# mushroomfire/mdapy

Hardware: AMD Instinct MI355X
Metric: atoms/sec for neighbor+CNA on 10M-atom FCC Cu; 1/2/4/8-GPU scaling (higher is better)
Workload: dtype f64 (CNA pair tests: f32 filter + f64 finish, labels exact); 1 GPU; FCC Cu a=3.615, 136^3 cells per GPU (10061824 atoms/GPU, 10061824 total), build_neighbor(rc=0.854a=3.08721, max_neigh=16) + fixed-cutoff CNA as one C-ABI call (mdh_build_neighbor_fcna: lists and labels), positions resident in HBM; atoms_per_gpu=10061824, max_neigh=16, parallelism=single, world_size_checked=1, launched_by=single process

## Files before the change

include/mdapy_amd.h:

```cpp
#ifndef MDAPY_AMD_H
#define MDAPY_AMD_H

#include <stdint.h>

#ifdef __cplusplus
extern "C" {
#endif

#define MDH_HOST 0
#define MDH_DEVICE 1

#define MDH_OK 0
#define MDH_ERR_BOX (-1)
#define MDH_ERR_HIP (-2)
#define MDH_ERR_ARG (-3)
#define MDH_ERR_NOMEM (-4)

const char *mdh_last_error(void);
int mdh_version(void);
int mdh_device_count(void);
int mdh_set_device(int device);
int mdh_warm(void);
int mdh_min_max_i32(const int *v, int64_t n, int *min_max2, int space, void *stream);
int mdh_dense_codes_i32(const int *v, int64_t n, int low, int span, int *codes, int64_t *counts_span, int space, void *stream);
int mdh_release_workspace(void);
int64_t mdh_workspace_bytes(void);
int mdh_prof_enable(int on);
int mdh_prof_reset(void);
int mdh_prof_report(char *buf, int buflen);
int mdh_debug_set_neighbor_variant(int variant);
int mdh_debug_set_indirect(int on);
int mdh_debug_set_slot_grid(int on);
int mdh_debug_slot_grid_counters(int64_t *out4);
int mdh_debug_slot_grid_rule(int ordered, int keyed, int windowed, int row_width, int64_t ncell, int64_t N, int seen, int big, int listed);
int mdh_debug_grid_plan(const int64_t *in24, const double *in6, int *out15);
int mdh_debug_neighbor_plan(int *plan8);
int mdh_debug_lane_plan(const int64_t *in_i, const double *in_d, const int *stats, double *out);
int mdh_debug_run_offset_table(int txy, int tz, unsigned *out3);
int mdh_debug_set_fcna_variant(int variant);
int mdh_debug_track_counters(int on);
int mdh_debug_counters(int64_t *out4);
int mdh_debug_set_rdf_variant(int variant);
int mdh_debug_set_knn_variant(int variant);
int mdh_debug_set_sq_variant(int variant);
int mdh_debug_set_entropy_variant(int variant);
int mdh_debug_set_ptm_order_cap(int cap);
int mdh_debug_image_thresholds(double L, double *out4);

int mdh_parse_table(const char *text, int64_t nbytes, int text_space, int64_t nrows, int ncol, const int *kinds,
                    void *const *columns, int64_t *redo, int64_t redo_cap, int64_t *status4, int space, void *stream);
int mdh_debug_text_pow5(int q, uint64_t *out2);
int mdh_debug_parse_double(const char *s, int64_t len, double *out);
int mdh_scan_sections(const char *text, int64_t nbytes, int text_space, const char *const *words, int nwords, int64_t *first_offset,
// ... 313 lines not shown
```

mdapy_amd/_lib.py:

```python
from __future__ import annotations

import ctypes as C
import os

import numpy as np

_HERE = os.path.dirname(os.path.abspath(__file__))
LIB_PATH = os.path.join(_HERE, "csrc", "libmdapy_amd.so")

HOST, DEVICE = 0, 1
ERR_BOX, ERR_HIP, ERR_ARG, ERR_NOMEM = -1, -2, -3, -4

_lib = None

i64, dbl, cint, vp = C.c_int64, C.c_double, C.c_int, C.c_void_p
ALLOC_ROWS = C.CFUNCTYPE(C.c_int, C.c_void_p, C.c_int64, C.c_int64, C.POINTER(C.POINTER(C.c_int)), C.POINTER(C.POINTER(C.c_double)))

_SIGNATURES = {
    "mdh_last_error": [],
    "mdh_version": [],
    "mdh_device_count": [],
    "mdh_set_device": [cint],
    "mdh_warm": [],
    "mdh_min_max_i32": [vp, i64, vp, cint, vp],
    "mdh_dense_codes_i32": [vp, i64, cint, cint, vp, vp, cint, vp],
    "mdh_release_workspace": [],
    "mdh_workspace_bytes": [],
    "mdh_prof_enable": [cint],
    "mdh_prof_reset": [],
    "mdh_prof_report": [vp, cint],
    "mdh_debug_set_neighbor_variant": [cint],
    "mdh_debug_set_indirect": [cint],
    "mdh_debug_set_slot_grid": [cint],
    "mdh_debug_slot_grid_counters": [vp],
    "mdh_debug_slot_grid_rule": [cint, cint, cint, cint, i64, i64, cint, cint, cint],
    "mdh_debug_grid_plan": [vp, vp, vp],
    "mdh_debug_neighbor_plan": [vp],
    "mdh_debug_lane_plan": [vp, vp, vp, vp],
    "mdh_debug_run_offset_table": [cint, cint, vp],
    "mdh_debug_set_fcna_variant": [cint],
    "mdh_debug_track_counters": [cint],
    "mdh_debug_counters": [vp],
    "mdh_debug_set_rdf_variant": [cint],
    "mdh_debug_set_knn_variant": [cint],
    "mdh_debug_set_sq_variant": [cint],
    "mdh_debug_set_entropy_variant": [cint],
    "mdh_debug_set_ptm_order_cap": [cint],
    "mdh_debug_image_thresholds": [dbl, vp],
    "mdh_parse_table": [vp, i64, cint, i64, cint, vp, vp, vp, i64, vp, cint, vp],
    "mdh_debug_text_pow5": [cint, vp],
    "mdh_debug_parse_double": [C.c_char_p, i64, vp],
    "mdh_scan_sections": [vp, i64, cint, vp, cint, vp, vp, vp],
    "mdh_debug_scan_sections": [vp, i64, vp, cint, vp, vp],
    "mdh_format_table": [i64, cint, vp, vp, vp, vp, vp, vp, i64, vp, vp, cint, vp],
# ... 192 lines not shown
```

mdapy_amd/csrc/neighbor_lane.hip:

```cpp
#include "common.hpp"
#include "grid.hpp"
#include "cna_core.hpp"
#include <algorithm>
#include <cassert>
#include <cmath>
#include <type_traits>
#include <cstdio>
#include <cstdlib>
#include <cstring>

namespace mdh {
namespace lane {

static constexpr int NEUTRAL = img::CELL_NEUTRAL;
static constexpr int NEUTRAL3 = img::NEUTRAL;

struct FastDiv {
    unsigned mul, sh1, sh2, d;
    __device__ __forceinline__ unsigned div(unsigned n) const
    {
        const unsigned t = __umulhi(mul, n);
        return (t + ((n - t) >> sh1)) >> sh2;
    }
};
// ... 28 lines not shown
}
static Shape make_shape(int txy, int tz, int nt1, int nt2)
{
    assert(txy >= 1 && tz >= 1 && (txy + 2) * (txy + 2) * (tz + 2) <= RUN_TABLE_HALO);
    assert(2 * run_offset(txy, tz, 8) <= RUN_TABLE_SPAN);
    Shape s{txy, tz, make_fastdiv((unsigned)nt2), make_fastdiv((unsigned)nt1), (65536u + (unsigned)tz + 1u) / ((unsigned)tz + 2u),
            (65536u + (unsigned)txy + 1u) / ((unsigned)txy + 2u), 0u, 0u, 0u};
    run_offset_table(txy, tz, &s.ro_lo, &s.ro_hi, &s.ro_bias);
    return s;
}
typedef __attribute__((address_space(3))) unsigned char lds_byte;
typedef int Int4 __attribute__((ext_vector_type(4)));

static thread_local int g_last_plan[8];
static thread_local int g_last_listed = -1;
#ifdef MDH_STAMPS
__device__ unsigned long long g_stamps[65536 * 8];
#define STAMP(k) do { if (tid == 0 && !parent && tile.id < 65536) g_stamps[tile.id * 8 + (k)] = __builtin_amdgcn_s_memtime(); } while (0)
#else
#define STAMP(k) do {} while (0)
#endif

__device__ __forceinline__ void lds_barrier()
{
    asm volatile("s_waitcnt lgkmcnt(0)\n\ts_barrier" ::: "memory");
}

__device__ __forceinline__ int excl_scan_block(int v, int *scratch, int *total)
{
    const int lane = threadIdx.x & 63, w = threadIdx.x >> 6;
// ... 93 lines not shown
                 "s_waitcnt lgkmcnt(2)\n\t" MDH_CAND2("v100", "v101", "v102", "v104", "v105", "v106")
                 "ds_read_b128 v[100:103], %[a] offset:128\n\t"
                 "ds_read_b128 v[104:107], %[a] offset:144\n\t"
                 "s_waitcnt lgkmcnt(2)\n\t" MDH_CAND2("v108", "v109", "v110", "v112", "v113", "v114")
                 "ds_read_b128 v[108:111], %[a] offset:160\n\t"
                 "ds_read_b128 v[112:115], %[a] offset:176\n\t"
                 "s_waitcnt lgkmcnt(2)\n\t" MDH_CAND2("v100", "v101", "v102", "v104", "v105", "v106")
                 "s_waitcnt lgkmcnt(0)\n\t" MDH_CAND2("v108", "v109", "v110", "v112", "v113", "v114")
                 : [m] "=&v"(m), [w] "+v"(w)
                 : [a] "v"(a), [sx] "v"(sx), [sy] "v"(sy), [sz] "v"(sz), [negc] "v"(negc)
                 : "memory", "v100", "v101", "v102", "v103", "v104", "v105", "v106", "v107", "v108", "v109", "v110", "v111", "v112", "v113",
                   "v114", "v115", "v116", "v117", "v118", "v119", "v120", "v121");
    mask = m;
}
#undef MDH_CAND2
__device__ __forceinline__ int run_slots(int len)
{
    return (len + 3) & ~3;
}

__device__ __forceinline__ bool sqrt_fast_ok(double x)
{
    return x >= 0x1p-767 && x < 0x1p+1000;
}
__device__ __forceinline__ bool sqrt_fast_ok4(const double (&x)[4])
{
    const unsigned h0 = (unsigned)__double2hiint(x[0]), h1 = (unsigned)__double2hiint(x[1]), h2 = (unsigned)__double2hiint(x[2]),
                   h3 = (unsigned)__double2hiint(x[3]);
    const unsigned lo = min(min(min(h0, h1), h2), h3), hi = max(max(max(h0, h1), h2), h3);
    return lo >= (256u << 20) && hi < (2023u << 20);
// ... 3 lines not shown
    const double y = __builtin_amdgcn_rsq(x);
    double g = x * y;
    double h = y * 0.5;
    const double r = __builtin_fma(-h, g, 0.5);
    g = __builtin_fma(g, r, g);
    h = __builtin_fma(h, r, h);
    const double d0 = __builtin_fma(-g, g, x);
    g = __builtin_fma(d0, h, g);
    const double d1 = __builtin_fma(-g, g, x);
    return __builtin_fma(d1, h, g);
}

template <bool SELF, bool TRI>
__device__ __forceinline__ unsigned scan_run_f64(const double2 *__restrict__ lxy, const double *__restrict__ lz,
                                                 const unsigned short *__restrict__ lsh, const DBox &b, double rcsq, int k0, int len,
                                                 int li, double xi, double yi, double zi)
{
    unsigned m = 0;
    const int S = run_slots(len);
    for (int j = 0; j < S; ++j) {
        const int k = k0 + j;
        bool h = false;
        if (j < len) {
            const double2 cj = lxy[k];
            const double d2 = exact_d2<TRI ? 2 : 1>(b, cj.x, cj.y, lz[k], xi, yi, zi, TRI ? 0 : lsh[k]);
            h = (d2 <= rcsq) && (!SELF || k != li);
        }
        m = m + m + (h ? 1u : 0u);
    }
    return m;
}

template <int NN, class Index>
__device__ __forceinline__ int lane_fcna_f32(Index index_of, const float4 *__restrict__ f4, float negc, float W)
{
    float ux[NN], uy[NN], uz[NN];
#pragma unroll
    for (int a = 0; a < NN; ++a) {
        const float4 c = f4[index_of(a)];
        ux[a] = c.x; uy[a] = c.y; uz[a] = c.z;
// ... 65 lines not shown
__device__ __forceinline__ CellGrid::Packed load_record(const CellGrid::Packed *__restrict__ pk, const IndirectSrc &src, int q, int coded)
{
    if (!IND)
        return pk[q];
    return load_atom(src, src.order[q], coded);
}

template <bool COUNT, bool TRI, bool LOOP, bool FCNA, bool TK8, bool IND = false, bool SLOT = false>
__global__ __launch_bounds__(NW * 64, (TK8 && (!FCNA || !LOOP)) ? 16 / NW : 1) void k_neighbor_lane(
    const CellGrid::Packed *__restrict__ pk, const int *__restrict__ cell_start, DBox b,
    Grid g, double rc, float negc, float W, int *__restrict__ verlet, double *__restrict__ dist, int *__restrict__ nn,
    int M, int write_pads, int cap, int *__restrict__ flags, unsigned char *__restrict__ tile_flag, int nt0,
    int nt1, int nt2, Shape ts, const int *__restrict__ tile_list, const int *__restrict__ n_live, int list_mode,
    int *__restrict__ max_count, int *__restrict__ flagged, const int *__restrict__ parent, int parent_nt2, int nsub,
    int flag_slot, int *__restrict__ pattern, int *__restrict__ cna_todo, int jt0, int rw, int tile_base, int *__restrict__ listed_sink,
    int cen_lo, int cen_hi, IndirectSrc isrc, int slot_hi)
{
    const int TXY = ts.txy, TZ = ts.tz;
    const int coded = IND ? flags[4] : 0;
    const int HXY = TXY + 2, HZ = TZ + 2, NH = HXY * HXY * HZ;

    extern __shared__ __attribute__((aligned(16))) unsigned char smem[];
    const int tid = threadIdx.x, lane = tid & 63;
    typedef typename std::conditional<TK8, unsigned char, unsigned short>::type Ticket;
    constexpr int JB = TK8 ? 5 : 8;
    float4 *f4 = reinterpret_cast<float4 *>(smem);
    double2 *lxy = reinterpret_cast<double2 *>(f4 + cap);
    double *lz = reinterpret_cast<double *>(lxy + cap);
    unsigned *cen = reinterpret_cast<unsigned *>(lz + cap);
    unsigned short *lsh = reinterpret_cast<unsigned short *>(cen + CEN_CAP);
    Ticket *tk = reinterpret_cast<Ticket *>(lsh + cap + (cap & 1));
    const unsigned f4_lds = (unsigned)(unsigned long)(lds_byte *)smem;
    const int TKS = ticket_row(M, false);
    const int wstride = max(rw * TKS, 256 / (int)sizeof(Ticket));
    auto hc = [&](int t) -> unsigned & { return reinterpret_cast<unsigned *>(tk + (size_t)(t >> 6) * wstride)[t & 63]; };
    __shared__ unsigned hr[NW * 64 + 2];
    __shared__ int scan_tmp[NW];
    __shared__ int s_flag[4];

    const double rcsq = rc * rc, pad = rc + 1.0;
    const double cw = rc;
    int vmax = 0;

    const int nlive = parent ? min(*n_live, nt0 * nt1 * parent_nt2) * nsub : ((list_mode && tile_list) ? *n_live : nt0 * nt1 * nt2);
    const int per = (nlive + 7) / 8;
// ... 85 lines not shown
    };
    for (int jt = jt0 + (int)(blockIdx.x >> 3); jt < per; jt += (int)(gridDim.x >> 3)) {
        const int slot = (int)(blockIdx.x & 7) * per + jt;
        if (slot >= nlive)
            break;
        const Tile tile = tile_of(slot);
        STAMP(0);
        Halo cur = halo_of(tile);
#ifdef MDH_STAMPS
        asm volatile("" : "+v"(cur.src), "+v"(cur.cnt));
        STAMP(1);
#endif
        double pa[4], pb[4], pc[4];
        int pd[4], pm[4];
        request(cur, pa, pb, pc, pd, pm);
        if (flags[0] != 0)
            return;
        const int tile_id = tile.id, T0 = tile.T0, T1 = tile.T1, T2 = tile.T2;
        const int cnt = cur.cnt, src = cur.src, img = cur.img, hz = cur.hz;
        const bool edge = cur.edge, centre_cell = cur.centre;
        if (tid == 0) { s_flag[0] = 0; s_flag[1] = 0; s_flag[2] = 0; s_flag[3] = 0; }
        hc(tid) = (unsigned)cnt;

        int total2;
        const int off2 = excl_scan_block(cnt | (centre_cell ? cnt << 16 : 0), scan_tmp, &total2);
        const int total = total2 & 0xffff, ncentres = total2 >> 16;
        const int off0 = off2 & 0xffff, coff = off2 >> 16;
        bool ok = !(total > cap || ncentres > CEN_CAP);
        const bool no_centres = ncentres == 0;
        if (no_centres) ok = false;
        if (SLOT && (img & 64)) s_flag[2] = 1;
        STAMP(2);
        if (ok && tid < NH && hz >= 1 && hz <= HZ - 2) {
            const unsigned k0 = (unsigned)off0 - hc(tid - 1), len = hc(tid - 1) + (unsigned)cnt + hc(tid + 1);
            hr[tid] = k0 | (len << 16);
            if (len > (TK8 ? 32u : 96u)) s_flag[2] = 1;
            if (TK8 && len > 12u) s_flag[3] = 1;
        }
        if (ok && cnt > 0) {
            double X0, Y0, Z0, XS, YS, ZS;
            const bool plain = !TRI && tile.interior;
            const int code0 = plain ? NEUTRAL3 : combine_codes(img, img::ATOM_NEUTRAL);
            if (TRI) {
                const double f0 = (double)(T0 - 1) * (cw / b.thick[0]) + (double)img::axis(code0, 0);
                const double f1 = (double)(T1 - 1) * (cw / b.thick[1]) + (double)img::axis(code0, 1);
                const double f2 = (double)(T2 - 1) * (cw / b.thick[2]) + (double)img::axis(code0, 2);
                XS = b.o[0] + f0 * b.h[0] + f1 * b.h[3] + f2 * b.h[6];
                YS = b.o[1] + f0 * b.h[1] + f1 * b.h[4] + f2 * b.h[7];
                ZS = b.o[2] + f0 * b.h[2] + f1 * b.h[5] + f2 * b.h[8];
                X0 = XS; Y0 = YS; Z0 = ZS;
            } else {
                X0 = b.o[0] + (double)(T0 - 1) * cw; Y0 = b.o[1] + (double)(T1 - 1) * cw; Z0 = b.o[2] + (double)(T2 - 1) * cw;
                if (plain) {
                    XS = X0; YS = Y0; ZS = Z0;
                } else {
                    XS = X0 + b.h[0] * (double)img::axis(code0, 0); YS = Y0 + b.h[4] * (double)img::axis(code0, 1);
                    ZS = Z0 + b.h[8] * (double)img::axis(code0, 2);
                }
            }
            const float flo = (float)(-1.5 * cw);
            const float fhx = (float)(((double)HXY + 1.5) * cw), fhz = (float)(((double)HZ + 1.5) * cw);
            bool general = code0 != NEUTRAL3, far = false;
            auto stage4 = [&](int k, const double (&a)[4], const double (&bb)[4], const double (&c)[4], const int (&d)[4], const int (&m)[4]) {
#pragma unroll
                for (int v = 0; v < 4; ++v) {
                    if (k + v < cnt) {
                        int code = code0;
                        float ux, uy, uz;
                        if (TRI) {
// ... 8 lines not shown
                                far = far || !(s0 >= -1.5 && s0 <= (double)HXY + 1.5 && s1 >= -1.5 && s1 <= (double)HXY + 1.5 && s2 >= -1.5 && s2 <= (double)HZ + 1.5);
                            }
                        } else {
                            ux = (float)(a[v] - XS); uy = (float)(bb[v] - YS); uz = (float)(c[v] - ZS);
                        }
                        if (!TRI && m[v] != img::ATOM_NEUTRAL) {
                            code = combine_codes(img, m[v]);
                            ux = (float)((a[v] - b.h[0] * (double)img::axis(code, 0)) - X0);
                            uy = (float)((bb[v] - b.h[4] * (double)img::axis(code, 1)) - Y0);
                            uz = (float)((c[v] - b.h[8] * (double)img::axis(code, 2)) - Z0);
                            general = true;
                        }
                        if (!TRI && edge)
                            far = far || !(ux >= flo && ux <= fhx && uy >= flo && uy <= fhx && uz >= flo && uz <= fhz);
                        const int p = off0 + k + v;
                        f4[p] = make_float4(ux, uy, uz, __int_as_float(d[v]));
                        lxy[p] = make_double2(a[v], bb[v]);
                        lz[p] = c[v];
                        lsh[p] = (unsigned short)code;
                        if (centre_cell) cen[coff + k + v] = (unsigned)p | ((unsigned)tid << 11);
                    }
                }
            };
            if (TK8) {
                for (int k = 0; k < cnt; k += 4) {
                    double a[4], bb[4], c[4];
                    int d[4], m[4];
#pragma unroll
                    for (int v = 0; v < 4; ++v) {
                        if (k == 0) { a[v] = pa[v]; bb[v] = pb[v]; c[v] = pc[v]; d[v] = pd[v]; m[v] = pm[v]; }
                        else {
                            const int kv = min(k + v, cnt - 1);
                            const int q = src + kv + (SLOT && kv >= 4 ? slot_hi : 0);
                            const CellGrid::Packed r = load_record<IND>(pk, isrc, q, coded);
// ... 23 lines not shown
                }
            }
            if (general) s_flag[0] = 1;
            if (far) s_flag[1] = 1;
        }
        __syncthreads();
        STAMP(3);
        if (ok && (s_flag[1] | s_flag[2]))
            ok = false;
        if (!ok && !no_centres && tid == 0) {
            if (tile_flag) tile_flag[tile_id] = 1;
            flagged[atomicAdd(&flags[flag_slot], 1)] = tile_id;
        }
        const bool general_tile = s_flag[0] != 0;
        const bool short_runs = TK8 && s_flag[3] == 0;
        const int wv = tid >> 6;
        Ticket *tkw = tk + (size_t)wv * wstride;
        const int A2 = HXY * HZ;
        auto run_cell = [&](int cbv, int r) {
            const int r3 = (r * 11) >> 5;
            return cbv + __mul24(r3, A2 - 3 * HZ) + __mul24(r, HZ) - (A2 + HZ);
        };
        constexpr unsigned R8 = TRI ? 8u : RUN8_SEL;
        auto run_at = [&](int cbv, unsigned cbk, unsigned sel) {
            return TRI ? run_cell(cbv, (int)sel) : (int)(cbk + __builtin_amdgcn_perm(ts.ro_hi, ts.ro_lo, sel));
        };
        for (int cbase = (int)((unsigned)(wv - jt) & (unsigned)(NW - 1)) * rw; ok && cbase < ncentres; cbase += NW * rw) {
            const int q = cbase + lane;
            const bool mine = lane < rw && q < ncentres;
            int kept = 0, kept8 = 0, cb = 0, id = 0;
            double xi = 0, yi = 0, zi = 0;
            Ticket *my = tkw + (size_t)lane * TKS;
            if (mine) {
                const unsigned cv = cen[q];
                const int li = (int)(cv & 2047u);
                cb = (int)(cv >> 11);
                const float4 s = f4[li];
                constexpr bool WIDE = !TK8;
                unsigned hv[9], mk[9], mk2[WIDE ? 9 : 1], mk3[WIDE ? 9 : 1];
#pragma unroll
                for (int r = 0; r < 9; ++r)
                    hv[r] = hr[cb + ((r / 3 - 1) * HXY + (r % 3 - 1)) * HZ];
                unsigned w = 0x7f7fffffu;
                if (TK8 && short_runs) {
#pragma unroll
                    for (int r = 0; r < 9; ++r) {
                        const int len = (int)(hv[r] >> 16);
                        scan_run12_asm(f4_lds + ((hv[r] & 0xffffu) << 4), s.x, s.y, s.z, negc, mk[r], w);
                        mk[r] = keep_top(mk[r] << 20, len);
                    }
                } else {
#pragma unroll
                    for (int r = 0; r < 9; ++r) {
                        const int len = (int)(hv[r] >> 16), la = WIDE ? min(len, 32) : len;
                        scan_run_asm(f4_lds + ((hv[r] & 0xffffu) << 4), la, s.x, s.y, s.z, negc, mk[r], w);
                        if (TK8)
                            mk[r] = and_not(mk[r] << ((32 - run_slots(la)) & 31), 0x7fffffffu >> ((la - 1) & 31));
                        else mk[r] &= ~0u << (run_slots(la) - la);
                        if (WIDE) {
                            const int lb = min(len - la, 32), lc = len - la - lb;
                            mk2[r] = 0;
                            mk3[r] = 0;
                            if (__builtin_amdgcn_ballot_w64(lb > 0)) {
                                scan_run_asm(f4_lds + (((hv[r] & 0xffffu) + 32u) << 4), lb, s.x, s.y, s.z, negc, mk2[r], w);
                                mk2[r] &= lb > 0 ? ~0u << (run_slots(lb) - lb) : 0u;
                                if (__builtin_amdgcn_ballot_w64(lc > 0)) {
                                    scan_run_asm(f4_lds + (((hv[r] & 0xffffu) + 64u) << 4), lc, s.x, s.y, s.z, negc, mk3[r], w);
                                    mk3[r] &= lc > 0 ? ~0u << (run_slots(lc) - lc) : 0u;
                                }
                            }
// ... 9 lines not shown
                }
                STAMP(4);
                {
                    const double2 ci = lxy[li];
                    xi = ci.x; yi = ci.y; zi = lz[li];
                    if (b.anypbc) {
                        if (TRI || general_tile) {
                            wrap<TRI>(b, xi, yi, zi);
                        } else {
                            if (b.pbc[0]) xi = b.o[0] + (xi - b.o[0]);
                            if (b.pbc[1]) yi = b.o[1] + (yi - b.o[1]);
                            if (b.pbc[2]) zi = b.o[2] + (zi - b.o[2]);
                        }
                    }
                }
                if (__builtin_expect(w <= __float_as_uint(W), 0)) {
#pragma unroll
                    for (int r = 0; r < 9; ++r) {
                        const int k0 = (int)(hv[r] & 0xffffu), len = (int)(hv[r] >> 16), la = WIDE ? min(len, 32) : len;
                        if (r == 4) mk[r] = scan_run_f64<true, TRI>(lxy, lz, lsh, b, rcsq, k0, la, li, xi, yi, zi);
                        else mk[r] = scan_run_f64<false, TRI>(lxy, lz, lsh, b, rcsq, k0, la, li, xi, yi, zi);
                        if (TK8) mk[r] <<= (32 - run_slots(la)) & 31;
                        if (WIDE) {
                            const int lb = min(len - la, 32), lc = len - la - lb;
                            if (r == 4) mk2[r] = scan_run_f64<true, TRI>(lxy, lz, lsh, b, rcsq, k0 + 32, lb, li, xi, yi, zi);
                            else mk2[r] = scan_run_f64<false, TRI>(lxy, lz, lsh, b, rcsq, k0 + 32, lb, li, xi, yi, zi);
                            if (r == 4) mk3[r] = scan_run_f64<true, TRI>(lxy, lz, lsh, b, rcsq, k0 + 64, lc, li, xi, yi, zi);
                            else mk3[r] = scan_run_f64<false, TRI>(lxy, lz, lsh, b, rcsq, k0 + 64, lc, li, xi, yi, zi);
                        }
                    }
                }
                int hits = 0;
#pragma unroll
                for (int r = 0; r < 9; ++r) hits += __builtin_popcount(mk[r]) + (WIDE ? __builtin_popcount(mk2[r]) + __builtin_popcount(mk3[r]) : 0);
                id = __float_as_int(s.w);
                nn[id] = hits;
                if (COUNT) {
                    vmax = max(vmax, hits);
                } else {
                    int sl = 0;
                    auto step = [&](unsigned &m, int jb) {
                        int z;
                        asm("v_ffbh_u32 %0, %1" : "=v"(z) : "v"(m));
                        const int none = z >> 31;
                        const unsigned slot = min((unsigned)(sl | none), (unsigned)M);
                        my[slot] = (Ticket)(jb + z);
                        sl += none + 1;
                        m &= ~(0x80000000u >> (z & 31));
                    };
#pragma unroll
// ... 65 lines not shown
                        for (int u = 0; u < 4; ++u) {
                            const int sx = g0 + u;
                            h[u] = sx < kept;
                            const unsigned t = (tw[sx >> 2] >> (8 * (sx & 3))) & 255u;
                            unsigned r = (sx >= kept - kept8) ? R8 : t >> 5;
                            r = h[u] ? r : 4u;
                            k[u] = (int)(hr[run_at(cb, cbk, r)] & 0xffffu) + (h[u] ? (int)(t & 31u) : 0);
                        }
                        double2 cj[4];
                        double zj[4], d2[4];
                        int nid[4], sh[4];
#pragma unroll
                        for (int u = 0; u < 4; ++u) {
                            cj[u] = lxy[k[u]];
                            zj[u] = lz[k[u]];
                            nid[u] = __float_as_int(f4[k[u]].w);
                            sh[u] = (!TRI && general_tile) ? (int)lsh[k[u]] : 0;
                        }
#pragma unroll
                        for (int u = 0; u < 4; ++u) {
                            if (TRI) d2[u] = exact_d2<2>(b, cj[u].x, cj[u].y, zj[u], xi, yi, zi, 0);
                            else if (general_tile) d2[u] = exact_d2<1>(b, cj[u].x, cj[u].y, zj[u], xi, yi, zi, sh[u]);
                            else d2[u] = exact_d2<0>(b, cj[u].x, cj[u].y, zj[u], xi, yi, zi, 0);
                            d2[u] = h[u] ? d2[u] : 1.0;
                        }
                        const bool slow = !sqrt_fast_ok4(d2);
                        double rr[4];
                        if (__builtin_expect(__builtin_amdgcn_ballot_w64(slow) == 0, 1)) {
#pragma unroll
                            for (int u = 0; u < 4; ++u) rr[u] = sqrt_fast(d2[u]);
                        } else {
// ... 299 lines not shown
    int *flagged2 = sc.alloc_n<int>((size_t)ntiles * (size_t)ll.nsub);
    if (sc.failed())
        return sc.error();
    hipStream_t st = sc.stream();
    if (ll.tiles == LaneLaunch::LIST) {
        hipLaunchKernelGGL(k_tile_live, dim3(grid_for(ntiles, 256)), dim3(256), 0, st, cg.cell_start, cg.g, nt[0], nt[1], nt[2], ts, live, cg.slot_cap);
        MDH_TRY(exclusive_scan_u32(sc, live, slot, ntiles));
        hipLaunchKernelGGL(k_tile_compact, dim3(grid_for(ntiles, 256)), dim3(256), 0, st, live, slot, (int)ntiles, tile_list);
    } else {
        tile_list = nullptr;
    }
    const dim3 grid(ll.grid);
    const size_t lds = (size_t)plan.lds_bytes;
    const int Mi = (int)M, wp = fill_pads ? (rows.ids_only ? 3 : 1) : 0;
    const float negc = -plan.mid;
    const dim3 grid2(SLICE_GRID);
    const Shape ts2 = make_shape(ts.txy, 1, nt[1], ll.nt2b);
    const bool indirect = !cg.pk;
    const lane::IndirectSrc isrc{cg.ix, cg.iy, cg.iz, cg.imv, cg.order};
    const int slot_hi = cg.slot_cap ? (int)(cg.slot_hi - 4) : 0;
#define MDH_LANE_PASS_I(COUNT, TRI, LOOP, FCNA, TK8, IND, SLOT, GRID, JT0, ...)                                                                 \
    do {                                                                                                                                  \
        if (lds > 60 * 1024)                             \
            (void)hipFuncSetAttribute(reinterpret_cast<const void *>(&k_neighbor_lane<COUNT, TRI, LOOP, FCNA, TK8, IND, SLOT>), hipFuncAttributeMaxDynamicSharedMemorySize, (int)lds); \
        hipLaunchKernelGGL((k_neighbor_lane<COUNT, TRI, LOOP, FCNA, TK8, IND, SLOT>), GRID, dim3(NW * 64), lds, st, cg.pk, cg.cell_start, b, \
                           cg.g, rc, negc, plan.T, verlet, dist, nn, Mi, wp, plan.cap, cg.flags, nullptr, __VA_ARGS__, pattern, tf.cna_todo, JT0, plan.rw, ll.tile_base, gs.listed_sink, \
                           ll.cen_lo, ll.cen_hi, isrc, slot_hi); \
    } while (0)
#define MDH_LANE_PASS(COUNT, TRI, LOOP, FCNA, TK8, GRID, JT0, ...)                                                                        \
    do {                                                                                                                                  \
        if (indirect && cg.slot_cap) MDH_LANE_PASS_I(COUNT, TRI, LOOP, FCNA, TK8, true, true, GRID, JT0, __VA_ARGS__);                    \
        else if (indirect) MDH_LANE_PASS_I(COUNT, TRI, LOOP, FCNA, TK8, true, false, GRID, JT0, __VA_ARGS__);                             \
        else MDH_LANE_PASS_I(COUNT, TRI, LOOP, FCNA, TK8, false, false, GRID, JT0, __VA_ARGS__);                                          \
    } while (0)
#define MDH_LANE_LAUNCH(COUNT, TRI, FCNA, TK8)                                                                                            \
    do {                                                                                                                                  \
        if (ll.tiles == LaneLaunch::LIST) {                                                                                               \
            MDH_LANE_PASS(COUNT, TRI, false, FCNA, TK8, grid, 0, nt[0], nt[1], nt[2], ts, tile_list, slot + ntiles, 1, max_count, flagged, nullptr, 0, 1, 2); \
            if (ll.standby)                                                                                                               \
                MDH_LANE_PASS(COUNT, TRI, true, FCNA, TK8, dim3(STANDBY_GRID), ll.per, nt[0], nt[1], nt[2], ts, tile_list, slot + ntiles, 1, max_count, flagged, nullptr, 0, 1, 2); \
        } else {                                                                                                                          \
            MDH_LANE_PASS(COUNT, TRI, false, FCNA, TK8, grid, 0, ll.nt0_run, nt[1], nt[2], ts, nullptr, slot + ntiles, 0, max_count, flagged, nullptr, 0, 1, 2); \
// ... 65 lines not shown
                             (double)p.occupied, (double)p.reason, (double)p.lds_bytes, (double)p.pop, (double)p.over96, (double)p.runs};
    std::copy(lane, lane + 15, out);
    std::copy(hook, hook + 8, out + 15);
    if (p.txy) {
        const LaneLaunch ll = plan_lane_launch(p, in.nc, (int)in_i[13], (int)in_i[14], (int)in_i[15], (int)in_i[16], gs.last_listed);
        const double launch[16] = {(double)ll.nt[0], (double)ll.nt[1], (double)ll.nt[2], (double)ll.ntiles, (double)ll.tiles, (double)ll.tile_base, (double)ll.nt0_run,
                                   (double)ll.per, (double)ll.grid, (double)ll.standby, (double)ll.slice_pass, (double)ll.nsub, (double)ll.nt2b, (double)ll.list_cap,
                                   (double)ll.mop_tile_z, (double)ll.mop_nt2};
        std::copy(launch, launch + 16, out + 23);
        out[44] = ll.cen_lo; out[45] = ll.cen_hi;
    }
    const TiledPlan tp = plan_tiled(ti);
    out[39] = tp.tile; out[40] = tp.tile_z; out[41] = tp.cellshift; out[42] = tp.full; out[43] = (double)tp.occupied;
    return MDH_OK;
}
extern "C" int mdh_debug_run_offset_table(int txy, int tz, unsigned *out3)
{
    if (txy < 1 || tz < 1 || (int64_t)(txy + 2) * (txy + 2) * (tz + 2) > mdh::lane::RUN_TABLE_HALO) return MDH_ERR_ARG;
    const mdh::lane::Shape s = mdh::lane::make_shape(txy, tz, 1, 1);
    out3[0] = s.ro_lo; out3[1] = s.ro_hi; out3[2] = s.ro_bias;
    return MDH_OK;
}

MDH_WARM_UNIT(neighbor_lane)
```

mdapy_amd/csrc/neighbor_plan.hpp:

```cpp
#pragma once
#include <stdint.h>
#include <stddef.h>
#include <algorithm>
#include <cmath>

#ifdef __HIPCC__
#define MDH_HD __host__ __device__
#else
#define MDH_HD
#endif

namespace mdh {

namespace img {
constexpr int MAX_M = 14;
}

struct GridStats {
    static constexpr int NBIN = 99;
    int v[NBIN];
    int last_listed = -1;
    int *listed_sink = nullptr;
};

namespace lane {

constexpr int NW = 4;
constexpr int CEN_CAP = 80 * NW;
MDH_HD constexpr int ticket_row(int M, bool cna_rows) { return (cna_rows && ((M + 4) & ~3) < 28) ? 28 : ((M + 4) & ~3); }
constexpr unsigned STANDBY_GRID = 512;
constexpr unsigned SLICE_GRID = 1024;

inline size_t lds_bytes(int cap, int64_t M, bool tk8, int rw, bool  = false)
{
    const size_t wave = std::max<size_t>((size_t)rw * (size_t)ticket_row((int)M, false) * (tk8 ? 1 : 2), 256);
    const size_t tk = (size_t)NW * wave;
    return (size_t)cap * 16 + (size_t)cap * 16 + (size_t)cap * 8 + (size_t)CEN_CAP * 4 + (size_t)(cap + (cap & 1)) * 2 + ((tk + 15) & ~(size_t)15);
}

}

struct LanePlanIn {
    int nc[3], mode;
    int pbc[3], tri;
    int64_t ncell;
    int64_t N, M;
    double h[9], o[3], thick[3];
    double rc;
    int fcna, count;
    int v[GridStats::NBIN];
    int zero_;
};
// ... 116 lines not shown
}

inline void lane_plan_hook(const LanePlanIn &, const LanePlan &p, int out8[8])
{
    for (int k = 0; k < 8; ++k) out8[k] = 0;
    if (!p.txy) {
        out8[6] = p.reason;
        if (p.reason == -5) { out8[5] = p.over96; out8[4] = p.runs; }
        if (p.reason == -7) out8[5] = p.pop;
        return;
    }
    out8[0] = p.txy; out8[1] = p.tz; out8[2] = p.cap; out8[3] = p.lds_bytes;
    out8[4] = p.full | (p.tk8 ? 2 : 0) | (p.wgs << 2); out8[5] = p.pop; out8[6] = (int)std::min<int64_t>(p.occupied, 2147483647); out8[7] = 1;
}

inline int expected_live_tiles_per_xcd(int64_t occupied, int cells_per_tile, int per_max)
{
    const int64_t est_live = std::max<int64_t>(1, occupied / std::max(1, cells_per_tile) * 2);
    return std::max(1, std::min(per_max, (int)((est_live + est_live / 4 + 7) / 8)));
}

struct LaneLaunch {
    enum Tiles { ALL, WINDOW, LIST };
    int nt[3];
    int64_t ntiles;
    Tiles tiles;
    int tile_base, nt0_run;
    int per;
    unsigned grid;
    bool standby;
// ... 159 lines not shown
```

Measured before the change: 7.857 billion atoms/s.

## Use expanded-distance f32 filter with precomputed norms on interior TK8 tiles

For interior tiles without image codes, the lane kernel now stores each candidate's squared norm in the float4 w slot, centred on the tile. The f32 filter evaluates |u|^2 - 2 s·u + (|s|^2 - mid) with fmac chains instead of subtracting coordinates. Atom ids move to a separate LDS array, and capacity shrinks to cap*42/44 to fit it. A rigorous rounding band (expanded_band) sets the threshold and the f64 fallback window, so labels stay exact. The change also adds debug counters for which layout ran, at the cost of an extra LDS indirection for ids and wider uncertain bands that may send more candidates to the f64 path.

```diff
diff --git a/include/mdapy_amd.h b/include/mdapy_amd.h
--- a/include/mdapy_amd.h
+++ b/include/mdapy_amd.h
@@ -37,6 +37,7 @@
 int mdh_debug_neighbor_plan(int *plan8);
 int mdh_debug_lane_plan(const int64_t *in_i, const double *in_d, const int *stats, double *out);
 int mdh_debug_run_offset_table(int txy, int tz, unsigned *out3);
+int mdh_debug_tile_layouts(int on, double *out10);
 int mdh_debug_set_fcna_variant(int variant);
 int mdh_debug_track_counters(int on);
 int mdh_debug_counters(int64_t *out4);
diff --git a/mdapy_amd/_lib.py b/mdapy_amd/_lib.py
--- a/mdapy_amd/_lib.py
+++ b/mdapy_amd/_lib.py
@@ -38,6 +38,7 @@
     "mdh_debug_neighbor_plan": [vp],
     "mdh_debug_lane_plan": [vp, vp, vp, vp],
     "mdh_debug_run_offset_table": [cint, cint, vp],
+    "mdh_debug_tile_layouts": [cint, vp],
     "mdh_debug_set_fcna_variant": [cint],
     "mdh_debug_track_counters": [cint],
     "mdh_debug_counters": [vp],
diff --git a/mdapy_amd/csrc/neighbor_lane.hip b/mdapy_amd/csrc/neighbor_lane.hip
--- a/mdapy_amd/csrc/neighbor_lane.hip
+++ b/mdapy_amd/csrc/neighbor_lane.hip
@@ -66,6 +66,8 @@
 
 static thread_local int g_last_plan[8];
 static thread_local int g_last_listed = -1;
+static int *g_lay_count = nullptr;
+static double g_lay_band[4] = {0, 0, 0, 0};
 #ifdef MDH_STAMPS
 __device__ unsigned long long g_stamps[65536 * 8];
 #define STAMP(k) do { if (tid == 0 && !parent && tile.id < 65536) g_stamps[tile.id * 8 + (k)] = __builtin_amdgcn_s_memtime(); } while (0)
@@ -189,6 +191,74 @@
     mask = m;
 }
 #undef MDH_CAND2
+#define MDH_CANDX2(X1, Y1, Z1, Q1, X2, Y2, Z2, Q2)                                                                                   \
+    "v_add_f32 v116, " Q1 ", %[k]\n\t"                                                                                               \
+    "v_add_f32 v119, " Q2 ", %[k]\n\t"                                                                                               \
+    "v_fmac_f32 v116, %[ax], " X1 "\n\t"                                                                                             \
+    "v_fmac_f32 v119, %[ax], " X2 "\n\t"                                                                                             \
+    "v_fmac_f32 v116, %[ay], " Y1 "\n\t"                                                                                             \
+    "v_fmac_f32 v119, %[ay], " Y2 "\n\t"                                                                                             \
+    "v_fmac_f32 v116, %[az], " Z1 "\n\t"                                                                                             \
+    "v_fmac_f32 v119, %[az], " Z2 "\n\t"                                                                                             \
+    "v_alignbit_b32 %[m], %[m], v116, 31\n\t"                                                                                        \
+    "v_alignbit_b32 %[m], %[m], v119, 31\n\t"                                                                                        \
+    "v_min3_u32 %[w], %[w], v116, v119\n\t"
+__device__ __forceinline__ void scan_runx_asm(unsigned a, int rem, float ax, float ay, float az, float k, unsigned &mask, unsigned &w)
+{
+    unsigned long long save;
+    unsigned m;
+    asm volatile("s_mov_b64 %[save], exec\n\t"
+                 "v_mov_b32 %[m], 0\n"
+                 ".Lscanx_top_%=:\n\t"
+                 "v_cmp_lt_i32 vcc, 0, %[rem]\n\t"
+                 "s_and_b64 exec, exec, vcc\n\t"
+                 "s_cbranch_execz .Lscanx_end_%=\n\t"
+                 "ds_read_b128 v[100:103], %[a]\n\t"
+                 "ds_read_b128 v[104:107], %[a] offset:16\n\t"
+                 "ds_read_b128 v[108:111], %[a] offset:32\n\t"
+                 "ds_read_b128 v[112:115], %[a] offset:48\n\t"
+                 "v_add_u32 %[a], 64, %[a]\n\t"
+                 "v_add_u32 %[rem], -4, %[rem]\n\t"
+                 "s_waitcnt lgkmcnt(2)\n\t" MDH_CANDX2("v100", "v101", "v102", "v103", "v104", "v105", "v106", "v107")
+                 "s_waitcnt lgkmcnt(0)\n\t" MDH_CANDX2("v108", "v109", "v110", "v111", "v112", "v113", "v114", "v115")
+                 "s_branch .Lscanx_top_%=\n"
+                 ".Lscanx_end_%=:\n\t"
+                 "s_mov_b64 exec, %[save]\n\t"
+                 : [m] "=&v"(m), [w] "+v"(w), [a] "+v"(a), [rem] "+v"(rem), [save] "=&s"(save)
+                 : [ax] "v"(ax), [ay] "v"(ay), [az] "v"(az), [k] "v"(k)
+                 : "vcc", "scc", "memory", "v100", "v101", "v102", "v103", "v104", "v105", "v106", "v107", "v108", "v109", "v110",
+                   "v111", "v112", "v113", "v114", "v115", "v116", "v117", "v118", "v119", "v120", "v121");
+    mask = m;
+}
+__device__ __forceinline__ void scan_run12x_asm(unsigned a, float ax, float ay, float az, float k, unsigned &mask, unsigned &w)
+{
+    unsigned m;
+    asm volatile("v_mov_b32 %[m], 0\n\t"
+                 "ds_read_b128 v[100:103], %[a]\n\t"
+                 "ds_read_b128 v[104:107], %[a] offset:16\n\t"
+                 "ds_read_b128 v[108:111], %[a] offset:32\n\t"
+                 "ds_read_b128 v[112:115], %[a] offset:48\n\t"
+                 "s_waitcnt lgkmcnt(2)\n\t" MDH_CANDX2("v100", "v101", "v102", "v103", "v104", "v105", "v106", "v107")
+                 "ds_read_b128 v[100:103], %[a] offset:64\n\t"
+                 "ds_read_b128 v[104:107], %[a] offset:80\n\t"
+                 "s_waitcnt lgkmcnt(2)\n\t" MDH_CANDX2("v108", "v109", "v110", "v111", "v112", "v113", "v114", "v115")
+                 "ds_read_b128 v[108:111], %[a] offset:96\n\t"
+                 "ds_read_b128 v[112:115], %[a] offset:112\n\t"
+                 "s_waitcnt lgkmcnt(2)\n\t" MDH_CANDX2("v100", "v101", "v102", "v103", "v104", "v105", "v106", "v107")
+                 "ds_read_b128 v[100:103], %[a] offset:128\n\t"
+                 "ds_read_b128 v[104:107], %[a] offset:144\n\t"
+                 "s_waitcnt lgkmcnt(2)\n\t" MDH_CANDX2("v108", "v109", "v110", "v111", "v112", "v113", "v114", "v115")
+                 "ds_read_b128 v[108:111], %[a] offset:160\n\t"
+                 "ds_read_b128 v[112:115], %[a] offset:176\n\t"
+                 "s_waitcnt lgkmcnt(2)\n\t" MDH_CANDX2("v100", "v101", "v102", "v103", "v104", "v105", "v106", "v107")
+                 "s_waitcnt lgkmcnt(0)\n\t" MDH_CANDX2("v108", "v109", "v110", "v111", "v112", "v113", "v114", "v115")
+                 : [m] "=&v"(m), [w] "+v"(w)
+                 : [a] "v"(a), [ax] "v"(ax), [ay] "v"(ay), [az] "v"(az), [k] "v"(k)
+                 : "memory", "v100", "v101", "v102", "v103", "v104", "v105", "v106", "v107", "v108", "v109", "v110", "v111", "v112", "v113",
+                   "v114", "v115", "v116", "v117", "v118", "v119", "v120", "v121");
+    mask = m;
+}
+#undef MDH_CANDX2
 __device__ __forceinline__ int run_slots(int len)
 {
     return (len + 3) & ~3;
@@ -222,7 +292,7 @@
 template <bool SELF, bool TRI>
 __device__ __forceinline__ unsigned scan_run_f64(const double2 *__restrict__ lxy, const double *__restrict__ lz,
                                                  const unsigned short *__restrict__ lsh, const DBox &b, double rcsq, int k0, int len,
-                                                 int li, double xi, double yi, double zi)
+                                                 int li, double xi, double yi, double zi, bool codes)
 {
     unsigned m = 0;
     const int S = run_slots(len);
@@ -231,7 +301,7 @@
         bool h = false;
         if (j < len) {
             const double2 cj = lxy[k];
-            const double d2 = exact_d2<TRI ? 2 : 1>(b, cj.x, cj.y, lz[k], xi, yi, zi, TRI ? 0 : lsh[k]);
+            const double d2 = exact_d2<TRI ? 2 : 1>(b, cj.x, cj.y, lz[k], xi, yi, zi, TRI ? 0 : (codes ? (int)lsh[k] : NEUTRAL3));
             h = (d2 <= rcsq) && (!SELF || k != li);
         }
         m = m + m + (h ? 1u : 0u);
@@ -327,8 +397,9 @@
     int nt1, int nt2, Shape ts, const int *__restrict__ tile_list, const int *__restrict__ n_live, int list_mode,
     int *__restrict__ max_count, int *__restrict__ flagged, const int *__restrict__ parent, int parent_nt2, int nsub,
     int flag_slot, int *__restrict__ pattern, int *__restrict__ cna_todo, int jt0, int rw, int tile_base, int *__restrict__ listed_sink,
-    int cen_lo, int cen_hi, IndirectSrc isrc, int slot_hi)
-{
+    int cen_lo, int cen_hi, IndirectSrc isrc, int slot_hi, float negcB, float WB, int capB, int *__restrict__ lay_count)
+{
+    constexpr bool CANB = TK8 && !TRI && !LOOP;
     const int TXY = ts.txy, TZ = ts.tz;
     const int coded = IND ? flags[4] : 0;
     const int HXY = TXY + 2, HZ = TZ + 2, NH = HXY * HXY * HZ;
@@ -338,10 +409,10 @@
     typedef typename std::conditional<TK8, unsigned char, unsigned short>::type Ticket;
     constexpr int JB = TK8 ? 5 : 8;
     float4 *f4 = reinterpret_cast<float4 *>(smem);
-    double2 *lxy = reinterpret_cast<double2 *>(f4 + cap);
-    double *lz = reinterpret_cast<double *>(lxy + cap);
-    unsigned *cen = reinterpret_cast<unsigned *>(lz + cap);
-    unsigned short *lsh = reinterpret_cast<unsigned short *>(cen + CEN_CAP);
+    double2 *const lxyA = reinterpret_cast<double2 *>(f4 + cap);
+    double *const lzA = reinterpret_cast<double *>(lxyA + cap);
+    unsigned *const cenA = reinterpret_cast<unsigned *>(lzA + cap);
+    unsigned short *lsh = reinterpret_cast<unsigned short *>(cenA + CEN_CAP);
     Ticket *tk = reinterpret_cast<Ticket *>(lsh + cap + (cap & 1));
     const unsigned f4_lds = (unsigned)(unsigned long)(lds_byte *)smem;
     const int TKS = ticket_row(M, false);
@@ -457,6 +528,7 @@
         double pa[4], pb[4], pc[4];
         int pd[4], pm[4];
         request(cur, pa, pb, pc, pd, pm);
+        const int any_code = CANB ? flags[4] : 0;
         if (flags[0] != 0)
             return;
         const int tile_id = tile.id, T0 = tile.T0, T1 = tile.T1, T2 = tile.T2;
@@ -472,6 +544,14 @@
         bool ok = !(total > cap || ncentres > CEN_CAP);
         const bool no_centres = ncentres == 0;
         if (no_centres) ok = false;
+        const bool expd = CANB && tile.interior && any_code == 0 && __builtin_amdgcn_readfirstlane(total) <= capB;
+        const int capL = expd ? capB : cap;
+        double2 *const lxy = CANB ? reinterpret_cast<double2 *>(f4 + capL) : lxyA;
+        double *const lz = CANB ? reinterpret_cast<double *>(lxy + capL) : lzA;
+        int *const idsB = reinterpret_cast<int *>(lz + capL);
+        unsigned *const cen = (CANB && expd) ? reinterpret_cast<unsigned *>(idsB + capL) : cenA;
+        const unsigned id_off = expd ? (unsigned)capL * 40u : 12u, id_sh = expd ? 2u : 4u;
+        auto id_at = [&](int k) { return *reinterpret_cast<const int *>(smem + id_off + ((unsigned)k << id_sh)); };
         if (SLOT && (img & 64)) s_flag[2] = 1;
         STAMP(2);
         if (ok && tid < NH && hz >= 1 && hz <= HZ - 2) {
@@ -496,6 +576,9 @@
                 X0 = b.o[0] + (double)(T0 - 1) * cw; Y0 = b.o[1] + (double)(T1 - 1) * cw; Z0 = b.o[2] + (double)(T2 - 1) * cw;
                 if (plain) {
                     XS = X0; YS = Y0; ZS = Z0;
+                    if (CANB && expd) {
+                        XS = X0 + 0.5 * (double)HXY * cw; YS = Y0 + 0.5 * (double)HXY * cw; ZS = Z0 + 0.5 * (double)HZ * cw;
+                    }
                 } else {
                     XS = X0 + b.h[0] * (double)img::axis(code0, 0); YS = Y0 + b.h[4] * (double)img::axis(code0, 1);
                     ZS = Z0 + b.h[8] * (double)img::axis(code0, 2);
@@ -534,10 +617,15 @@
                         if (!TRI && edge)
                             far = far || !(ux >= flo && ux <= fhx && uy >= flo && uy <= fhx && uz >= flo && uz <= fhz);
                         const int p = off0 + k + v;
-                        f4[p] = make_float4(ux, uy, uz, __int_as_float(d[v]));
+                        if (CANB && expd) {
+                            f4[p] = make_float4(ux, uy, uz, expanded_q(ux, uy, uz));
+                            idsB[p] = d[v];
+                        } else {
+                            f4[p] = make_float4(ux, uy, uz, __int_as_float(d[v]));
+                            lsh[p] = (unsigned short)code;
+                        }
                         lxy[p] = make_double2(a[v], bb[v]);
                         lz[p] = c[v];
-                        lsh[p] = (unsigned short)code;
                         if (centre_cell) cen[coff + k + v] = (unsigned)p | ((unsigned)tid << 11);
                     }
                 }
@@ -591,6 +679,10 @@
         }
         const bool general_tile = s_flag[0] != 0;
         const bool short_runs = TK8 && s_flag[3] == 0;
+        if (CANB && lay_count && ok && tid == 0) {
+            atomicAdd(&lay_count[expd ? 1 : 0], 1);
+            atomicAdd(&lay_count[expd ? 3 : 2], (ncentres + 63) >> 6);
+        }
         const int wv = tid >> 6;
         Ticket *tkw = tk + (size_t)wv * wstride;
         const int A2 = HXY * HZ;
@@ -619,18 +711,36 @@
                 for (int r = 0; r < 9; ++r)
                     hv[r] = hr[cb + ((r / 3 - 1) * HXY + (r % 3 - 1)) * HZ];
                 unsigned w = 0x7f7fffffu;
+                const float c0 = (CANB && expd) ? -2.0f * s.x : s.x, c1 = (CANB && expd) ? -2.0f * s.y : s.y, c2 = (CANB && expd) ? -2.0f * s.z : s.z;
+                const float c3 = (CANB && expd) ? expanded_k(s.w, negcB) : negc;
                 if (TK8 && short_runs) {
+                    if (CANB && expd) {
+#pragma unroll
+                        for (int r = 0; r < 9; ++r) {
+                            const int len = (int)(hv[r] >> 16);
+                            scan_run12x_asm(f4_lds + ((hv[r] & 0xffffu) << 4), c0, c1, c2, c3, mk[r], w);
+                            mk[r] = keep_top(mk[r] << 20, len);
+                        }
+                    } else {
 #pragma unroll
                     for (int r = 0; r < 9; ++r) {
                         const int len = (int)(hv[r] >> 16);
-                        scan_run12_asm(f4_lds + ((hv[r] & 0xffffu) << 4), s.x, s.y, s.z, negc, mk[r], w);
+                        scan_run12_asm(f4_lds + ((hv[r] & 0xffffu) << 4), c0, c1, c2, c3, mk[r], w);
                         mk[r] = keep_top(mk[r] << 20, len);
+                    }
+                    }
+                } else if (CANB && expd) {
+#pragma unroll
+                    for (int r = 0; r < 9; ++r) {
+                        const int len = (int)(hv[r] >> 16);
+                        scan_runx_asm(f4_lds + ((hv[r] & 0xffffu) << 4), len, c0, c1, c2, c3, mk[r], w);
+                        mk[r] = and_not(mk[r] << ((32 - run_slots(len)) & 31), 0x7fffffffu >> ((len - 1) & 31));
                     }
                 } else {
 #pragma unroll
                     for (int r = 0; r < 9; ++r) {
                         const int len = (int)(hv[r] >> 16), la = WIDE ? min(len, 32) : len;
-                        scan_run_asm(f4_lds + ((hv[r] & 0xffffu) << 4), la, s.x, s.y, s.z, negc, mk[r], w);
+                        scan_run_asm(f4_lds + ((hv[r] & 0xffffu) << 4), la, c0, c1, c2, c3, mk[r], w);
                         if (TK8)
                             mk[r] = and_not(mk[r] << ((32 - run_slots(la)) & 31), 0x7fffffffu >> ((la - 1) & 31));
                         else mk[r] &= ~0u << (run_slots(la) - la);
@@ -670,26 +780,28 @@
                         }
                     }
                 }
-                if (__builtin_expect(w <= __float_as_uint(W), 0)) {
+                if (__builtin_expect(w <= __float_as_uint((CANB && expd) ? WB : W), 0)) {
+                    if (CANB && lay_count && lane == (int)__builtin_ctzll(__builtin_amdgcn_ballot_w64(true)))
+                        atomicAdd(&lay_count[expd ? 5 : 4], 1);
 #pragma unroll
                     for (int r = 0; r < 9; ++r) {
                         const int k0 = (int)(hv[r] & 0xffffu), len = (int)(hv[r] >> 16), la = WIDE ? min(len, 32) : len;
-                        if (r == 4) mk[r] = scan_run_f64<true, TRI>(lxy, lz, lsh, b, rcsq, k0, la, li, xi, yi, zi);
-                        else mk[r] = scan_run_f64<false, TRI>(lxy, lz, lsh, b, rcsq, k0, la, li, xi, yi, zi);
+                        if (r == 4) mk[r] = scan_run_f64<true, TRI>(lxy, lz, lsh, b, rcsq, k0, la, li, xi, yi, zi, !expd);
+                        else mk[r] = scan_run_f64<false, TRI>(lxy, lz, lsh, b, rcsq, k0, la, li, xi, yi, zi, !expd);
                         if (TK8) mk[r] <<= (32 - run_slots(la)) & 31;
                         if (WIDE) {
                             const int lb = min(len - la, 32), lc = len - la - lb;
-                            if (r == 4) mk2[r] = scan_run_f64<true, TRI>(lxy, lz, lsh, b, rcsq, k0 + 32, lb, li, xi, yi, zi);
-                            else mk2[r] = scan_run_f64<false, TRI>(lxy, lz, lsh, b, rcsq, k0 + 32, lb, li, xi, yi, zi);
-                            if (r == 4) mk3[r] = scan_run_f64<true, TRI>(lxy, lz, lsh, b, rcsq, k0 + 64, lc, li, xi, yi, zi);
-                            else mk3[r] = scan_run_f64<false, TRI>(lxy, lz, lsh, b, rcsq, k0 + 64, lc, li, xi, yi, zi);
+                            if (r == 4) mk2[r] = scan_run_f64<true, TRI>(lxy, lz, lsh, b, rcsq, k0 + 32, lb, li, xi, yi, zi, !expd);
+                            else mk2[r] = scan_run_f64<false, TRI>(lxy, lz, lsh, b, rcsq, k0 + 32, lb, li, xi, yi, zi, !expd);
+                            if (r == 4) mk3[r] = scan_run_f64<true, TRI>(lxy, lz, lsh, b, rcsq, k0 + 64, lc, li, xi, yi, zi, !expd);
+                            else mk3[r] = scan_run_f64<false, TRI>(lxy, lz, lsh, b, rcsq, k0 + 64, lc, li, xi, yi, zi, !expd);
                         }
                     }
                 }
                 int hits = 0;
 #pragma unroll
                 for (int r = 0; r < 9; ++r) hits += __builtin_popcount(mk[r]) + (WIDE ? __builtin_popcount(mk2[r]) + __builtin_popcount(mk3[r]) : 0);
-                id = __float_as_int(s.w);
+                id = CANB ? id_at(li) : __float_as_int(s.w);
                 nn[id] = hits;
                 if (COUNT) {
                     vmax = max(vmax, hits);
@@ -785,7 +897,7 @@
                         for (int u = 0; u < 4; ++u) {
                             cj[u] = lxy[k[u]];
                             zj[u] = lz[k[u]];
-                            nid[u] = __float_as_int(f4[k[u]].w);
+                            nid[u] = CANB ? id_at(k[u]) : __float_as_int(f4[k[u]].w);
                             sh[u] = (!TRI && general_tile) ? (int)lsh[k[u]] : 0;
                         }
 #pragma unroll
@@ -1115,6 +1227,13 @@
     const size_t lds = (size_t)plan.lds_bytes;
     const int Mi = (int)M, wp = fill_pads ? (rows.ids_only ? 3 : 1) : 0;
     const float negc = -plan.mid;
+    const ExpandedBand xb = expanded_band(lane_plan_in(b, cg.g, N, M, gs, rc, false, count), plan);
+    const int capB = expanded_cap(plan.cap);
+    int *const lay_count = g_lay_count;
+    if (lay_count) {
+        MDH_HIP(hipMemsetAsync(lay_count, 0, 6 * sizeof(int), st));
+        g_lay_band[0] = (double)capB; g_lay_band[1] = (double)xb.mid; g_lay_band[2] = (double)xb.T; g_lay_band[3] = xb.tol;
+    }
     const dim3 grid2(SLICE_GRID);
     const Shape ts2 = make_shape(ts.txy, 1, nt[1], ll.nt2b);
     const bool indirect = !cg.pk;
@@ -1126,7 +1245,7 @@
             (void)hipFuncSetAttribute(reinterpret_cast<const void *>(&k_neighbor_lane<COUNT, TRI, LOOP, FCNA, TK8, IND, SLOT>), hipFuncAttributeMaxDynamicSharedMemorySize, (int)lds); \
         hipLaunchKernelGGL((k_neighbor_lane<COUNT, TRI, LOOP, FCNA, TK8, IND, SLOT>), GRID, dim3(NW * 64), lds, st, cg.pk, cg.cell_start, b, \
                            cg.g, rc, negc, plan.T, verlet, dist, nn, Mi, wp, plan.cap, cg.flags, nullptr, __VA_ARGS__, pattern, tf.cna_todo, JT0, plan.rw, ll.tile_base, gs.listed_sink, \
-                           ll.cen_lo, ll.cen_hi, isrc, slot_hi); \
+                           ll.cen_lo, ll.cen_hi, isrc, slot_hi, -xb.mid, xb.T, capB, lay_count); \
     } while (0)
 #define MDH_LANE_PASS(COUNT, TRI, LOOP, FCNA, TK8, GRID, JT0, ...)                                                                        \
     do {                                                                                                                                  \
@@ -1222,6 +1341,26 @@
     out[39] = tp.tile; out[40] = tp.tile_z; out[41] = tp.cellshift; out[42] = tp.full; out[43] = (double)tp.occupied;
     return MDH_OK;
 }
+extern "C" int mdh_debug_tile_layouts(int on, double *out10)
+{
+    using namespace mdh;
+    for (int k = 0; k < 10; ++k) out10[k] = -1.0;
+    if (lane::g_lay_count) {
+        int h[6] = {0, 0, 0, 0, 0, 0};
+        MDH_HIP(hipMemcpy(h, lane::g_lay_count, sizeof(h), hipMemcpyDeviceToHost));
+        out10[0] = h[0]; out10[1] = h[1];
+        for (int k = 0; k < 4; ++k) out10[2 + k] = lane::g_lay_band[k];
+        for (int k = 0; k < 4; ++k) out10[6 + k] = h[2 + k];
+    }
+    if (on && !lane::g_lay_count) {
+        MDH_HIP(hipMalloc(reinterpret_cast<void **>(&lane::g_lay_count), 6 * sizeof(int)));
+        MDH_HIP(hipMemset(lane::g_lay_count, 0, 6 * sizeof(int)));
+    } else if (!on && lane::g_lay_count) {
+        (void)hipFree(lane::g_lay_count);
+        lane::g_lay_count = nullptr;
+    }
+    return MDH_OK;
+}
 extern "C" int mdh_debug_run_offset_table(int txy, int tz, unsigned *out3)
 {
     if (txy < 1 || tz < 1 || (int64_t)(txy + 2) * (txy + 2) * (tz + 2) > mdh::lane::RUN_TABLE_HALO) return MDH_ERR_ARG;
diff --git a/mdapy_amd/csrc/neighbor_plan.hpp b/mdapy_amd/csrc/neighbor_plan.hpp
--- a/mdapy_amd/csrc/neighbor_plan.hpp
+++ b/mdapy_amd/csrc/neighbor_plan.hpp
@@ -36,6 +36,15 @@
     const size_t wave = std::max<size_t>((size_t)rw * (size_t)ticket_row((int)M, false) * (tk8 ? 1 : 2), 256);
     const size_t tk = (size_t)NW * wave;
     return (size_t)cap * 16 + (size_t)cap * 16 + (size_t)cap * 8 + (size_t)CEN_CAP * 4 + (size_t)(cap + (cap & 1)) * 2 + ((tk + 15) & ~(size_t)15);
+}
+
+MDH_HD constexpr int expanded_cap(int cap) { return (int)(((long)cap * 42) / 44); }
+
+MDH_HD inline float expanded_q(float ux, float uy, float uz) { return __builtin_fmaf(uz, uz, __builtin_fmaf(uy, uy, ux * ux)); }
+MDH_HD inline float expanded_k(float qs, float negmid) { return qs + negmid; }
+MDH_HD inline float expanded_e(float q, float K, float ax, float ay, float az, float ux, float uy, float uz)
+{
+    return __builtin_fmaf(az, uz, __builtin_fmaf(ay, uy, __builtin_fmaf(ax, ux, q + K)));
 }
 
 }
@@ -182,6 +191,35 @@
     out8[4] = p.full | (p.tk8 ? 2 : 0) | (p.wgs << 2); out8[5] = p.pop; out8[6] = (int)std::min<int64_t>(p.occupied, 2147483647); out8[7] = 1;
 }
 
+struct ExpandedBand { float mid, T; double tol; double U2, S2; };
+inline ExpandedBand expanded_band(const LanePlanIn &in, const LanePlan &p)
+{
+    ExpandedBand e{0.0f, 0.0f, 0.0, 0.0, 0.0};
+    if (!p.txy || in.tri)
+        return e;
+    const double rc = in.rc, rcsq = rc * rc, eps = std::ldexp(1.0, -24);
+    double U2 = 0, S2 = 0, big = 0;
+    for (int d = 0; d < 3; ++d) {
+        const int T = d == 2 ? p.tz : p.txy;
+        const double extra = in.pbc[d] ? std::max(0.0, in.thick[d] - (double)in.nc[d] * rc) : 0.0;
+        const double hu = (0.5 * (double)(T + 2) + 1.0 / 64.0) * rc + extra, hs = (0.5 * (double)T + 1.0 / 64.0) * rc;
+        U2 += hu * hu;
+        S2 += hs * hs;
+        big = std::max(big, std::fabs(in.o[d]) + 2.0 * std::fabs(in.h[d * 4]));
+    }
+    const double U = std::sqrt(U2), S = std::sqrt(S2);
+    const double A = 1.02 * eps * (3.0 * U2 + 3.0 * S2 + (S2 + rcsq) + (U2 + S2 + rcsq) + 3.0 * ((U + S) * (U + S) + rcsq));
+    const double dd = 1.02 * eps * (U + S) + std::ldexp(big, -48);
+    const double tol = A + 2.0 * rc * dd + dd * dd;
+    float c = (float)(rcsq - tol);
+    while ((double)c > rcsq - tol) c = std::nextafterf(c, -INFINITY);
+    const double want = (rcsq - (double)c) + tol;
+    float W = (float)want;
+    while ((double)W < want) W = std::nextafterf(W, INFINITY);
+    e.mid = c; e.T = W; e.tol = tol; e.U2 = U2; e.S2 = S2;
+    return e;
+}
+
 inline int expected_live_tiles_per_xcd(int64_t occupied, int cells_per_tile, int per_max)
 {
     const int64_t est_live = std::max<int64_t>(1, occupied / std::max(1, cells_per_tile) * 2);
```

Result: no change. 7.801 billion atoms/s (-0.7%).
